# zubair-irshad/articulated-object-nerf

Measured on AMD Instinct MI355X. Metric: rays/sec (64c+128f samples), higher is better.
Workload: dtype f32; 1 GPU; sapien-single-scene vanilla NeRF full-frame render 640x480, 65 coarse + 193 fine evals/ray, 307200 rays per GPU per step, randomized=False, white_bkgd=True; rays_per_gpu=307200, evals_per_ray=258, exchange=none

## Files before the change

### articulated-object-nerf_amd/csrc/aon_mlp.hip

```cpp
#include "aon_pass.h"

namespace aon {

struct VanillaNet {
  static constexpr int kSlotBytes = kPairSlotBytes;
  static constexpr bool kPair = true;
  static constexpr int kNumChunks = aon::kNumChunks;
  static constexpr int chunk_bytes(int c) { return aon::chunk_bytes(c); }
};
struct VanillaFoldNet {
  static constexpr int kSlotBytes = kPairSlotBytes;
  static constexpr bool kPair = true;
  static constexpr int kNumChunks = aon::kNumChunksF;
  static constexpr int chunk_bytes(int c) { return aon::chunk_bytes_f(c); }
};
struct VanillaFoldVbNet {
  static constexpr int kSlotBytes = kPairSlotBytes;
  static constexpr bool kPair = true;
  static constexpr int kNumChunks = aon::kNumChunksF - 1;
  static constexpr int chunk_bytes(int c) { return aon::chunk_bytes_f(c < kChFView ? c : c + 1); }
  static constexpr int skip_before(int c) { return c == kChFView ? kSmallChunkBytes : 0; }
};

struct VanillaTrunkNet {
  static constexpr int kSlotBytes = kPairSlotBytes;
  static constexpr bool kPair = true;
  static constexpr int kNumChunks = kChBott;
  static constexpr int chunk_bytes(int) { return kBigChunkBytes; }
};

struct PackArgs {
  const float* p[kNumVanillaParams];
};

template <bool FOLD>
__global__ void pack_vanilla_kernel(PackArgs a, float* __restrict__ packed, int L, int Lv) {
  const int P = 3 + 6 * L, V = 3 + 6 * Lv;
  const int64_t idx = (int64_t)blockIdx.x * blockDim.x + threadIdx.x;
  constexpr int64_t stream_floats = kStreamBytes / 4;
  constexpr int64_t used_floats = FOLD ? kStreamBytesF / 4 : stream_floats;
  const float* Wf = packed + kFoldTmpOff / 4;
  if (idx >= stream_floats + kSmallFloats) return;
  if (idx >= used_floats && idx < stream_floats) {
    if (idx >= used_floats + 128 * 256 + 128) packed[idx] = 0.f;
    return;
  }
  if (idx >= stream_floats) {
    const int s = (int)(idx - stream_floats);
    float v = 0.f;
    if (s < kSmBiasBott) v = a.p[2 * (s >> 8) + 1][s & 255];
    else if (s < kSmBiasView) v = a.p[19][s - kSmBiasBott];
    else if (s < kSmWSigma) v = FOLD ? Wf[128 * 256 + s - kSmBiasView] : a.p[17][s - kSmBiasView];
    else if (s < kSmWRgb) v = a.p[20][s - kSmWSigma];
    else if (s < kSmBSigma) v = a.p[22][s - kSmWRgb];
    else if (s < kSmBRgb) v = a.p[21][0];
    else if (s < kSmBRgb + 3) v = a.p[23][s - kSmBRgb];
    packed[idx] = v;
    return;
  }
  int c, r, nt;
  constexpr int nbig = FOLD ? kChFView : kNumBigChunks;
  if (idx < (int64_t)nbig * (kBigChunkBytes / 4)) {
    c = (int)(idx / (kBigChunkBytes / 4)); r = (int)(idx % (kBigChunkBytes / 4)); nt = 8;
  } else {
    const int64_t i2 = idx - (int64_t)nbig * (kBigChunkBytes / 4);
    c = nbig + (int)(i2 / (kSmallChunkBytes / 4)); r = (int)(i2 % (kSmallChunkBytes / 4)); nt = 4;
    if constexpr (FOLD) c = c == kChFView ? kChView + 8 : c - 1 + (kChView - kChFView);
  }
  const int cc = r & 3, lane = (r >> 2) & 63, rest = r >> 8;
  const int tp = rest % nt, q = rest / nt;
  const int h = lane >> 5, row = 32 * tp + (lane & 31);
  const float* W; int ld, n_out = 256, col;
  const int hid_col = 8 * q + 4 * h + cc;
  auto pcol = [&](int c63) { return c63 < 0 ? -1 : pos_col_in(c63, L); };
  auto vcol = [&](int c27) { return c27 < 0 ? -1 : view_col_in(c27, Lv); };
  if (c < kChL1) { W = a.p[0]; ld = P; col = pcol(posenc_col(c, q, cc, h)); }
  else if (c < kChL5) { const int l = 1 + (c - kChL1) / 8; W = a.p[2 * l]; ld = 256; col = 32 * ((c - kChL1) % 8) + hid_col; }
  else if (c < kChL5 + 8) { W = a.p[10]; ld = 256 + P; col = 32 * (c - kChL5) + hid_col; }
  else if (c < kChL6) { W = a.p[10]; ld = 256 + P; col = pcol(posenc_col(c - kChL5 - 8, q, cc, h)); if (col >= 0) col += 256; }
  else if (c < kChL7) { W = a.p[12]; ld = 256; col = 32 * (c - kChL6) + hid_col; }
  else if (c < kChBott) { W = a.p[14]; ld = 256; col = 32 * (c - kChL7) + hid_col; }
  else if (c < kChView) { W = a.p[18]; ld = 256; col = 32 * (c - kChBott) + hid_col; }
  else if (c < kChView + 8) {
    W = a.p[16]; ld = 256 + V; n_out = kCondWidth; col = 32 * (c - kChView) + hid_col;
    if constexpr (FOLD) { W = Wf; ld = 256; }
  }
  else { W = a.p[16]; ld = 256 + V; n_out = kCondWidth; col = vcol(viewenc_col(q, cc, h)); if (col >= 0) col += 256; }
  packed[idx] = (col >= 0 && row < n_out) ? W[(int64_t)row * ld + col] : 0.f;
}

struct MlpSeg {
  const char* packed;
  const float* rays_o;
  const float* rays_d;
  const float* viewdirs;
  const float* t_vals;
  const float* samples_enc;
  const float* viewdirs_enc;
  float* raw;
  int64_t total;
  int S;
  int npass;
  union {
    float* planes;
    const int* gather_idx;
    float* live_rows;
  };
  union {
    u32x4* masks;
    const int64_t* gather_count;
    uint8_t* live_mark;
  };
  int64_t Np;
  const float* view_bias;
  static constexpr bool kPerCallBlock = false;
};
struct MlpArgs {
  MlpSeg seg[2];
  int npass_total;
};
__host__ __device__ __forceinline__ const char* seg_stream(const MlpSeg& s) { return s.packed; }
__device__ __forceinline__ const float* seg_small(const MlpSeg& s) { return reinterpret_cast<const float*>(s.packed + kStreamBytes); }

constexpr int kLdsBytes = kRingBytes + (int)kSmallBytes;

struct VanillaTrunk {
  static constexpr int kL0 = kChL0, kL1 = kChL1, kL5 = kChL5, kL6 = kChL6, kL7 = kChL7;
  static constexpr int kBias = kSmBias, kWSigma = kSmWSigma, kBSigma = kSmBSigma, kMask0 = 0;
  static constexpr int plane(int l) { return plane_h(l); }
};

template <bool ENC_IN_KERNEL, bool TRAIN, bool FOLD, bool VB = false, bool GATHER = false, bool DEFER = false>
__global__ void __launch_bounds__(256) mlp_fwd_kernel(MlpArgs args) {
  static_assert(FOLD || !VB, "the per-ray view bias belongs to the folded form");
  static_assert(!GATHER || (ENC_IN_KERNEL && !TRAIN), "the occupancy list serves the inference kernel on in-kernel encodings");
  static_assert(!DEFER || (ENC_IN_KERNEL && !TRAIN && VB && !GATHER), "the deferred view branch serves the dense per-ray-bias inference form");
  using Net = std::conditional_t<DEFER, VanillaTrunkNet, std::conditional_t<VB, VanillaFoldVbNet, std::conditional_t<FOLD, VanillaFoldNet, VanillaNet>>>;
  const int tid = threadIdx.x;
  const int lane = tid & 63, wave = tid >> 6;
  const int m = lane & 31, h = lane >> 5;
  const int wave_s = __builtin_amdgcn_readfirstlane(wave);

  run_passes<Net, kSmallFloats, GATHER>(args, [&](const MlpSeg& sg, int pass, Pipe& p, const float* sm, int64_t listed = 0) __attribute__((always_inline)) {
    int64_t g = (int64_t)pass * 128 + wave * 32 + m;
    bool valid;
    int64_t gc;
    if constexpr (GATHER) {
      valid = g < listed;
      g = gc = sg.gather_idx[valid ? g : listed - 1];
    } else {
      valid = g < sg.total;
      gc = valid ? g : sg.total - 1;
    }
    const int64_t ray = gc / sg.S;

    f32x16 E[2], V;
    float x[3] = {0.f, 0.f, 0.f}, vd[3] = {0.f, 0.f, 0.f};
    if constexpr (ENC_IN_KERNEL) {
      const float t = sg.t_vals[gc];
#pragma unroll
      for (int a = 0; a < 3; ++a) {
        x[a] = __fadd_rn(sg.rays_o[ray * 3 + a], __fmul_rn(t, sg.rays_d[ray * 3 + a]));
        vd[a] = sg.viewdirs[ray * 3 + a];
      }
      encode_pos(x, h, E);
      if constexpr (!VB || TRAIN) encode_view(vd, h, V);
    } else {
      load_pos_enc(sg.samples_enc + gc * kPosEnc, h, E);
      if constexpr (!VB || TRAIN) load_view_enc(sg.viewdirs_enc + ray * kViewEnc, h, V);
    }
    int ray32 = (int)ray;
    (void)ray32;

    PlaneIO io{};
    unsigned moff = 0;
    if constexpr (TRAIN) { io = make_plane_io(sg.planes, kPlRows, (int64_t)pass * 4 + wave_s, m, h); moff = mask_lane_off(pass, tid); }
    if constexpr (TRAIN) {
      store_pos_enc_plane(E, io, kPlE, h);
      store_view_enc_plane(V, io, kPlVE, h);
    }
    FwdTaps<TRAIN, MlpSeg> taps{sg, io, moff};
    f32x16 X[8], Y[8], Z[4];
    auto reread_enc = [&]() {
      if constexpr (TRAIN && !ENC_IN_KERNEL) {
        int64_t gq = gc;
        asm volatile("" : "+v"(gq));
        load_pos_enc(sg.samples_enc + gq * kPosEnc, h, E);
      }
    };
    auto l7_side = [&](auto plain) {
      if constexpr (VB && !DEFER) {
        asm volatile("" : "+v"(ray32));
        return view_bias_side(plain, sg.view_bias + (int64_t)ray32 * kCondWidth + 4 * h, Z);
      } else {
        return plain;
      }
    };
    const float sigma = trunk_fwd<Net, VanillaTrunk>(p, E, X, Y, sm, h, taps, reread_enc, l7_side);
    if constexpr (DEFER) {
      const bool live = sigma > 0.f;
      if (valid) {
        if (h == 0) {
          f32x4 o; o[0] = 0.f; o[1] = 0.f; o[2] = 0.f; o[3] = sigma;
          reinterpret_cast<f32x4*>(sg.raw)[g] = o;
          sg.live_mark[g] = live ? 1 : 0;
        }
        if (live) {
          char* row = reinterpret_cast<char*>(sg.live_rows) + g * 1024 + h * 16;
#pragma unroll
          for (int t = 0; t < 8; ++t) {
#pragma unroll
            for (int q = 0; q < 4; ++q) {
              f32x4 v; v[0] = Y[t][4 * q]; v[1] = Y[t][4 * q + 1]; v[2] = Y[t][4 * q + 2]; v[3] = Y[t][4 * q + 3];
              __builtin_nontemporal_store(v, reinterpret_cast<f32x4*>(row + (32 * t + 8 * q) * 4));
            }
          }
        }
      }
    } else {
      constexpr int kChV = FOLD ? kChFView : kChView;
      auto reencode_view = [&]() {
        if constexpr (TRAIN && ENC_IN_KERNEL) {
          asm volatile("" : "+v"(vd[0]), "+v"(vd[1]), "+v"(vd[2]));
          encode_view(vd, h, V);
        }
        if constexpr (TRAIN && !ENC_IN_KERNEL) {
          int64_t rq = ray;
          asm volatile("" : "+v"(rq));
          load_view_enc(sg.viewdirs_enc + rq * kViewEnc, h, V);
        }
      };
      if constexpr (FOLD) {
        if constexpr (!VB) {
          init_bias(Z, sm + kSmBiasView, h);
          reencode_view();
          chunk_mma<Net, kChV, 4, 14>(p, V, Z);
        }
        dense_layer<Net, kChV + (VB ? 0 : 1), 8, 4>(p, Y, Z, taps.consume(Y, plane_h(7), true)); taps.put_mask(7);
      } else {
        init_bias(X, sm + kSmBiasBott, h); dense_layer<Net, kChBott, 8, 8>(p, Y, X, taps.consume(Y, plane_h(7), true)); taps.put_mask(7);
        init_bias(Z, sm + kSmBiasView, h);
        dense_layer<Net, kChV, 8, 4>(p, X, Z, taps.consume(X, kPlBot, false));
        reencode_view();
        chunk_mma<Net, kChV + 8, 4, 14>(p, V, Z);
      }
      relu_tiles(Z);
      taps.burst(Z, kPlHV, 8);
      float rgb[3];
#pragma unroll
      for (int ch = 0; ch < 3; ++ch) {
        float v = head_partial<4>(Z, sm + kSmWRgb + ch * kCondWidth, h);
        rgb[ch] = v + __shfl_xor(v, 32) + sm[kSmBRgb + ch];
      }
      if (valid && h == 0) {
        f32x4 o; o[0] = rgb[0]; o[1] = rgb[1]; o[2] = rgb[2]; o[3] = sigma;
        reinterpret_cast<f32x4*>(sg.raw)[g] = o;
      }
    }
  });
}

void vanilla_fold_jobs_fwd(const float* const* params, float* packed, int view_levels, FoldGemm jobs[2]) {
  float* Wf = packed + kFoldTmpOff / 4;
  fold_view_jobs(params[16], 256 + 3 + 6 * view_levels, params[17], params[18], params[19], Wf, Wf + 128 * 256, jobs);
}

hipError_t launch_pack_vanilla(const float* const* params, float* packed, hipStream_t stream, int pos_levels, int view_levels, bool fold_done) {
  PackArgs a;
  for (int i = 0; i < kNumVanillaParams; ++i) a.p[i] = params[i];
  const int64_t n = kStreamBytes / 4 + kSmallFloats;
  const int form = fold_default();
  set_stream_form(packed, form);
  if (form == kFormFolded) {
    if (!fold_done) {
      FoldGemm jobs[2];
      vanilla_fold_jobs_fwd(params, packed, view_levels, jobs);
      if (hipError_t e = launch_fold_gemms(jobs, 2, stream); e != hipSuccess) return e;
    }
    pack_vanilla_kernel<true><<<dim3((unsigned)((n + 255) / 256)), dim3(256), 0, stream>>>(a, packed, pos_levels, view_levels);
  } else {
    pack_vanilla_kernel<false><<<dim3((unsigned)((n + 255) / 256)), dim3(256), 0, stream>>>(a, packed, pos_levels, view_levels);
  }
  return hipGetLastError();
}

int num_cus() {
  static std::atomic<int> cache[kMaxDevices];
  int dev = 0;
  if (hipGetDevice(&dev) != hipSuccess) return -1;
  if (dev < 0 || dev >= kMaxDevices) return -1;
  int cus = cache[dev].load(std::memory_order_relaxed);
  if (cus == 0) {
    hipDeviceProp_t prop;
    if (hipGetDeviceProperties(&prop, dev) != hipSuccess) return -1;
    cus = prop.multiProcessorCount;
    cache[dev].store(cus, std::memory_order_relaxed);
  }
  return cus;
}

template <bool ENC, bool TRAIN, bool FOLD, bool VB = false, bool GATHER = false, bool DEFER = false>
static hipError_t launch_mlp_tf(const MlpArgs& args, hipStream_t stream) {
  static DeviceOnce lds_once;
  return launch_persistent(&mlp_fwd_kernel<ENC, TRAIN, FOLD, VB, GATHER, DEFER>, kLdsBytes, args.npass_total, lds_once, stream, args);
}

template <bool ENC, bool TRAIN, bool GATHER = false>
static hipError_t launch_mlp_t(const MlpArgs& args, hipStream_t stream) {
  const int form = agreed_form(args);
  if (form == kFormUnknown) return hipErrorInvalidValue;
  if (args.seg[0].view_bias != nullptr) {
    if constexpr (ENC) return launch_mlp_tf<ENC, TRAIN, true, true, GATHER>(args, stream);
    else return hipErrorInvalidValue;
  }
  return form == kFormFolded ? launch_mlp_tf<ENC, TRAIN, true, false, GATHER>(args, stream)
                             : launch_mlp_tf<ENC, TRAIN, false, false, GATHER>(args, stream);
}

__global__ __launch_bounds__(256) void view_bias_kernel(const float* chunk, const float* bias_vec, const float* viewdirs, int64_t n_rays, float* out) {
  __shared__ float enc[8][2][16];
  const int tid = threadIdx.x;
  const int64_t ray0 = (int64_t)blockIdx.x * 8;
  if (tid < 16) {
    const int64_t ray = ray0 + (tid >> 1);
    if (ray < n_rays) {
      float vd[3] = {viewdirs[ray * 3], viewdirs[ray * 3 + 1], viewdirs[ray * 3 + 2]};
      f32x16 V;
      encode_view(vd, tid & 1, V);
#pragma unroll
      for (int r = 0; r < 16; ++r) enc[tid >> 1][tid & 1][r] = V[r];
    }
  }
  const int row = tid & 127, tp = row >> 5;
  const float bias = bias_vec[row];
  float w[14][2];
#pragma unroll
  for (int r = 0; r < 14; ++r)
#pragma unroll
    for (int hh = 0; hh < 2; ++hh) w[r][hh] = chunk[((((r >> 2) * 4 + tp) * 64 + hh * 32 + (row & 31)) << 2) + (r & 3)];
  __syncthreads();
  for (int k = tid >> 7; k < 8; k += 2) {
    const int64_t ray = ray0 + k;
    if (ray >= n_rays) break;
    float acc = bias;
#pragma unroll
    for (int r = 0; r < 14; ++r) {
      acc = __builtin_fmaf(w[r][0], enc[k][0][r], acc);
      acc = __builtin_fmaf(w[r][1], enc[k][1][r], acc);
    }
    out[ray * kCondWidth + row] = acc;
  }
}

hipError_t launch_view_bias_raw(const float* chunk, const float* bias_vec, const float* viewdirs, int64_t n_rays, float* out, hipStream_t stream) {
  if (n_rays <= 0) return hipSuccess;
  view_bias_kernel<<<dim3((unsigned)((n_rays + 7) / 8)), dim3(256), 0, stream>>>(chunk, bias_vec, viewdirs, n_rays, out);
  return hipGetLastError();
}

hipError_t launch_view_bias(const char* packed, const float* viewdirs, int64_t n_rays, float* out, hipStream_t stream) {
  if (stream_form(packed) != kFormFolded) return hipErrorInvalidValue;
  return launch_view_bias_raw(reinterpret_cast<const float*>(packed + chunk_offset_f(kChFView)), reinterpret_cast<const float*>(packed + kStreamBytes) + kSmBiasView,
                              viewdirs, n_rays, out, stream);
}

struct ViewArgs {
  const char* packed;
  const float* rows;
  const int* idx;
  const int64_t* count;
  const float* view_bias;
  float* raw;
  int S;
};
constexpr int kViewWBytes = 8 * kSmallChunkBytes;
constexpr int kViewLdsBytes = kViewWBytes + (int)kSmallBytes;

__device__ __forceinline__ int view_listed(const ViewArgs& a, int64_t listed, int64_t tile, int m) {
  const int64_t e = tile * 32 + m;
  return a.idx[e < listed ? e : listed - 1];
}
__device__ __forceinline__ void view_gather_tile(const ViewArgs& a, int g, int h, int t, f32x16& Y) {
  const char* row = reinterpret_cast<const char*>(a.rows) + (int64_t)g * 1024 + h * 16;
#pragma unroll
  for (int q = 0; q < 4; ++q) {
    const f32x4 v = *reinterpret_cast<const f32x4*>(row + (32 * t + 8 * q) * 4);
    Y[4 * q] = v[0]; Y[4 * q + 1] = v[1]; Y[4 * q + 2] = v[2]; Y[4 * q + 3] = v[3];
  }
}
__device__ __forceinline__ void view_bias_init(const ViewArgs& a, int g, int h, f32x16 (&Z)[4]) {
  const float* vb = a.view_bias + (int64_t)(g / a.S) * kCondWidth + 4 * h;
#pragma unroll
  for (int i = 0; i < 16; ++i) {
    const f32x4 v = *reinterpret_cast<const f32x4*>(vb + 32 * (i >> 2) + 8 * (i & 3));
    Z[i >> 2][4 * (i & 3)] = v[0]; Z[i >> 2][4 * (i & 3) + 1] = v[1]; Z[i >> 2][4 * (i & 3) + 2] = v[2]; Z[i >> 2][4 * (i & 3) + 3] = v[3];
  }
}
__device__ __forceinline__ void view_chunk(const char* w, int j, int lane, const f32x16& Y, f32x16 (&Z)[4], const f32x16 (&Z0)[4]) {
  const char* buf = w + j * kSmallChunkBytes + lane * 16;
#pragma unroll
  for (int i = 0; i < 16; ++i) {
    const int q = i / 4, tp = i % 4;
    const f32x4 av = *reinterpret_cast<const f32x4*>(buf + i * 1024);
#pragma unroll
    for (int cc = 0; cc < 4; ++cc)
      Z[tp] = __builtin_amdgcn_mfma_f32_32x32x2f32(av[cc], Y[4 * q + cc], (j == 0 && q == 0 && cc == 0) ? Z0[tp] : Z[tp], 0, 0, 0);
  }
}

__global__ void __launch_bounds__(256) view_kernel(ViewArgs a) {
  extern __shared__ __attribute__((aligned(16))) char smem[];
  const int64_t listed = *a.count;
  const int64_t ntiles = (listed + 31) / 32;
  if ((int64_t)blockIdx.x * 4 >= ntiles) return;
  float* sm = reinterpret_cast<float*>(smem + kViewWBytes);
  {
    const f32x4* src = reinterpret_cast<const f32x4*>(a.packed + chunk_offset_f(kChFView + 1));
    f32x4* dst = reinterpret_cast<f32x4*>(smem);
    for (int i = threadIdx.x; i < kViewWBytes / 16; i += 256) dst[i] = src[i];
  }
  load_small_block<kSmallFloats>(sm, reinterpret_cast<const float*>(a.packed + kStreamBytes));
  __syncthreads();
  const int lane = threadIdx.x & 63, m = lane & 31, h = lane >> 5;
  const int wave = __builtin_amdgcn_readfirstlane(threadIdx.x >> 6);
  const int64_t stride = (int64_t)gridDim.x * 4;
  int64_t tile = (int64_t)blockIdx.x * 4 + wave;
  if (tile >= ntiles) return;
  f32x16 Y[8], Z[4], Zb[4];
  int g = view_listed(a, listed, tile, m);
  int gn = view_listed(a, listed, tile + stride, m);
  __builtin_amdgcn_sched_barrier(0);
  view_bias_init(a, g, h, Zb);
  __builtin_amdgcn_sched_barrier(0);
#pragma unroll
  for (int t = 0; t < 8; ++t) view_gather_tile(a, g, h, t, Y[t]);
  __builtin_amdgcn_sched_barrier(0);
  while (true) {
    const int64_t nxt = tile + stride;
    const int gnn = view_listed(a, listed, nxt + stride, m);
#pragma unroll
    for (int j = 0; j < 8; ++j) {
      view_chunk(smem, j, lane, Y[j], Z, Zb);
      __builtin_amdgcn_sched_barrier(0);
      view_gather_tile(a, gn, h, j, Y[j]);
      if (j == 3) view_bias_init(a, gn, h, Zb);
      __builtin_amdgcn_sched_barrier(0);
    }
    relu_tiles(Z);
    float rgb[3];
#pragma unroll
    for (int ch = 0; ch < 3; ++ch) {
      const float v = head_partial<4>(Z, sm + kSmWRgb + ch * kCondWidth, h);
      rgb[ch] = v + __shfl_xor(v, 32) + sm[kSmBRgb + ch];
    }
    if (tile * 32 + m < listed && h == 0) {
      float* rec = a.raw + (int64_t)g * 4;
      rec[0] = rgb[0]; rec[1] = rgb[1]; rec[2] = rgb[2];
    }
    if (nxt >= ntiles) break;
    tile = nxt; g = gn; gn = gnn;
  }
}

hipError_t launch_mlp_trunk_defer(const char* packed, const float* rays_o, const float* rays_d, const float* viewdirs, const float* t_vals,
                                  int64_t n_rays, int S, float* raw, uint8_t* live_mark, float* live_rows, hipStream_t stream) {
  if (stream_form(packed) != kFormFolded) return hipErrorInvalidValue;
  MlpArgs args{};
  fill_seg(args.seg[0], TrainSeg{packed, nullptr, rays_o, rays_d, viewdirs, t_vals, n_rays, S, raw, nullptr, nullptr, 0, nullptr});
  args.seg[0].live_rows = live_rows; args.seg[0].live_mark = live_mark;
  finish_segs(args, 1);
  return launch_mlp_tf<true, false, true, true, false, true>(args, stream);
}

hipError_t launch_view_deferred(const char* packed, const float* live_rows, const int* idx, const int64_t* count, int64_t max_listed,
                                const float* view_bias, int S, float* raw, hipStream_t stream) {
  if (stream_form(packed) != kFormFolded) return hipErrorInvalidValue;
  if (max_listed <= 0) return hipSuccess;
  static DeviceOnce lds_once;
  if (hipError_t e = set_max_lds(&view_kernel, kViewLdsBytes, lds_once); e != hipSuccess) return e;
  const int cus = num_cus();
  if (cus <= 0) return hipErrorInvalidDevice;
  const int64_t groups = (max_listed + 127) / 128;
  const ViewArgs a{packed, live_rows, idx, count, view_bias, raw, S};
  view_kernel<<<dim3((unsigned)(groups < cus ? groups : cus)), dim3(256), kViewLdsBytes, stream>>>(a);
  return hipGetLastError();
}

hipError_t launch_mlp_fwd(const char* packed, const float* rays_o, const float* rays_d, const float* viewdirs,
                          const float* t_vals, int64_t n_rays, int S, float* raw, hipStream_t stream, const float* view_bias) {
  MlpArgs args{};
  fill_seg(args.seg[0], TrainSeg{packed, nullptr, rays_o, rays_d, viewdirs, t_vals, n_rays, S, raw, nullptr, nullptr, 0, view_bias});
  finish_segs(args, 1);
  return launch_mlp_t<true, false>(args, stream);
}

hipError_t launch_mlp_fwd_gather(const char* packed, const float* rays_o, const float* rays_d, const float* viewdirs, const float* t_vals,
                                 int64_t n_rays, int S, float* raw, hipStream_t stream, const float* view_bias, const int* idx, const int64_t* count,
                                 int64_t max_listed) {
  MlpArgs args{};
  MlpSeg& a = args.seg[0];
  fill_seg(a, TrainSeg{packed, nullptr, rays_o, rays_d, viewdirs, t_vals, n_rays, S, raw, nullptr, nullptr, 0, view_bias});
  if (max_listed > 0) a.npass = (int)((max_listed + 127) / 128);
  a.gather_idx = idx; a.gather_count = count;
  finish_segs(args, 1);
  return launch_mlp_t<true, false, true>(args, stream);
}

hipError_t launch_mlp_fwd_train(const char* packed, const float* rays_o, const float* rays_d, const float* viewdirs,
                                const float* t_vals, int64_t n_rays, int S, float* raw, float* planes, void* masks,
                                hipStream_t stream, int64_t np_total, const float* view_bias) {
  const TrainSeg one{packed, nullptr, rays_o, rays_d, viewdirs, t_vals, n_rays, S, raw, planes, masks, np_total, view_bias};
  return launch_mlp_fwd_train2(&one, 1, stream);
}

hipError_t launch_mlp_fwd_train2(const TrainSeg* segs, int nsegs, hipStream_t stream) {
  if (nsegs < 1 || nsegs > 2) return hipErrorInvalidValue;
  MlpArgs args{};
  for (int i = 0; i < nsegs; ++i) fill_seg(args.seg[i], segs[i]);
  finish_segs(args, nsegs);
  return launch_mlp_t<true, true>(args, stream);
}

hipError_t launch_mlp_fwd_train_enc(const char* packed, const float* samples_enc, const float* viewdirs_enc, int64_t n_rays, int S, float* raw,
                                    float* planes, void* masks, hipStream_t stream, int64_t np_total) {
  MlpArgs args{};
  fill_seg(args.seg[0], TrainSeg{packed, nullptr, nullptr, nullptr, nullptr, nullptr, n_rays, S, raw, planes, masks, np_total});
  args.seg[0].samples_enc = samples_enc; args.seg[0].viewdirs_enc = viewdirs_enc;
  finish_segs(args, 1);
  return launch_mlp_t<false, true>(args, stream);
}

hipError_t launch_mlp_fwd_enc(const char* packed, const float* samples_enc, const float* viewdirs_enc,
                              int64_t n_rays, int S, float* raw, hipStream_t stream) {
  MlpArgs args{};
  fill_seg(args.seg[0], TrainSeg{packed, nullptr, nullptr, nullptr, nullptr, nullptr, n_rays, S, raw, nullptr, nullptr, 0});
  args.seg[0].samples_enc = samples_enc; args.seg[0].viewdirs_enc = viewdirs_enc;
  finish_segs(args, 1);
  return launch_mlp_t<false, false>(args, stream);
}


__global__ void __launch_bounds__(256) density_grid_kernel(GridArgs args) {
  const int lane = threadIdx.x & 63, wave = threadIdx.x >> 6;
  const int m = lane & 31, h = lane >> 5;
  run_passes_one<VanillaTrunkNet, kSmallFloats>(args.packed, reinterpret_cast<const float*>(args.packed + kStreamBytes), args.npass,
                                                [&](int pass, Pipe& p, const float* sm) __attribute__((always_inline)) {
    const int64_t l0 = (int64_t)pass * 128 + wave * 32;
    const int64_t l = l0 + m;
    float x[3];
    grid_point(args, l < args.total ? l : args.total - 1, x);
    f32x16 E[2], X[8], Y[8];
    encode_pos(x, h, E);
    NoTaps taps;
    const float sigma = trunk_fwd<VanillaTrunkNet, VanillaTrunk>(p, E, X, Y, sm, h, taps);
    grid_store(args.out, l0, args.total, lane, grid_activation(sigma, args.act));
  });
}

hipError_t launch_density_grid(const char* packed, const int64_t* dims, const float* lo, const float* step, int64_t g_begin, int64_t g_end,
                               int act, float* out, hipStream_t stream) {
  if (stream_form(packed) == kFormUnknown) return hipErrorInvalidValue;
// ... 7 lines not shown
```

### articulated-object-nerf_amd/csrc/aon_mlp_core.h

```cpp
#pragma once
#include "aon_common.h"

#include <type_traits>

namespace aon {

constexpr int kPairSlotBytes = 2 * kBigChunkBytes;
constexpr int kRingBytes = 2 * kPairSlotBytes;

template <class Net> constexpr int pair_offset(int C) { return (C & 1) ? Net::chunk_bytes(C - 1) : 0; }
template <class Net> constexpr int dma_count(int C) {
  return (Net::kNumChunks & 1) ? (C == Net::kNumChunks - 1 ? 2 : (C == Net::kNumChunks - 2 ? 0 : 1)) : 1;
}
template <class Net> constexpr int dma_target(int C, int k) {
  return ((Net::kNumChunks & 1) && C == Net::kNumChunks - 1) ? k : (C + 2) % Net::kNumChunks;
}

template <class Net, class = void> struct NetSkip { static constexpr int at(int) { return 0; } };
template <class Net> struct NetSkip<Net, std::void_t<decltype(Net::skip_before(0))>> { static constexpr int at(int c) { return Net::skip_before(c); } };

struct Pipe {
  const char* stream;
  const char* next_stream;
  char* ring;
// ... 100 lines not shown
    if constexpr (ROUNDS > 0) {
      if (i < ROUNDS) dma_round<Net, C>(p, dma_off, i);
    }
    constexpr int SIDE_PER_STEP = NSTEP >= 16 ? 1 : (16 + NSTEP - 1) / NSTEP;
#pragma unroll
    for (int k = 0; k < SIDE_PER_STEP; ++k) side(i * SIDE_PER_STEP + k);
#pragma unroll
    for (int cc = 0; cc < 4; ++cc) {
      if (4 * q + cc < NREG) {
        if (ZERO_C && q == 0 && cc == 0) {
          const f32x16 zero = {0.f, 0.f, 0.f, 0.f, 0.f, 0.f, 0.f, 0.f, 0.f, 0.f, 0.f, 0.f, 0.f, 0.f, 0.f, 0.f};
          out[tp] = __builtin_amdgcn_mfma_f32_32x32x2f32(a_cur[cc], in[4 * q + cc], zero, 0, 0, 0);
        } else {
          out[tp] = __builtin_amdgcn_mfma_f32_32x32x2f32(a_cur[cc], in[4 * q + cc], out[tp], 0, 0, 0);
        }
      }
    }
    a_cur = a_nxt;
  }
}

template <int NT_OUT>
__device__ __forceinline__ void init_bias(f32x16 (&acc)[NT_OUT], const float* sm_bias, int h) {
#pragma unroll
  for (int tp = 0; tp < NT_OUT; ++tp) {
#pragma unroll
    for (int g = 0; g < 4; ++g) {
      const f32x4 b = *reinterpret_cast<const f32x4*>(sm_bias + 32 * tp + 8 * g + 4 * h);
      acc[tp][4 * g + 0] = b[0]; acc[tp][4 * g + 1] = b[1]; acc[tp][4 * g + 2] = b[2]; acc[tp][4 * g + 3] = b[3];
    }
  }
}

__device__ __forceinline__ float relu1(float x) {
  const int b = __builtin_bit_cast(int, x);
  return __builtin_bit_cast(float, b > 0 ? b : 0);
}

template <int NT>
__device__ __forceinline__ void relu_tiles(f32x16 (&x)[NT]) {
#pragma unroll
  for (int t = 0; t < NT; ++t) {
#pragma unroll
    for (int r = 0; r < 16; ++r) {
      float y = relu1(x[t][r]);
      asm("" : "+v"(y));
      x[t][r] = y;
    }
  }
}

struct NoSideOf {
  __device__ __forceinline__ NoSide operator()(int) const { return NoSide{}; }
};

template <class Net, int CBASE, int NT_IN, int NT_OUT, class SideOf = NoSideOf, bool ZERO_OUT = false>
__device__ __forceinline__ void dense_layer(Pipe& p, const f32x16 (&in)[NT_IN], f32x16 (&out)[NT_OUT], SideOf side_of = SideOf{}) {
  chunk_mma<Net, CBASE + 0, NT_OUT, 16, decltype(side_of(0)), ZERO_OUT>(p, in[0], out, side_of(0));
  chunk_mma<Net, CBASE + 1, NT_OUT, 16>(p, in[1], out, side_of(1));
  chunk_mma<Net, CBASE + 2, NT_OUT, 16>(p, in[2], out, side_of(2));
  chunk_mma<Net, CBASE + 3, NT_OUT, 16>(p, in[3], out, side_of(3));
  if constexpr (NT_IN == 8) {
    chunk_mma<Net, CBASE + 4, NT_OUT, 16>(p, in[4], out, side_of(4));
    chunk_mma<Net, CBASE + 5, NT_OUT, 16>(p, in[5], out, side_of(5));
    chunk_mma<Net, CBASE + 6, NT_OUT, 16>(p, in[6], out, side_of(6));
    chunk_mma<Net, CBASE + 7, NT_OUT, 16>(p, in[7], out, side_of(7));
  }
}

template <int NT>
__device__ __forceinline__ float head_partial(const f32x16 (&x)[NT], const float* sm_w, int h) {
  float acc = 0.f;
#pragma unroll
  for (int t = 0; t < NT; ++t) {
#pragma unroll
    for (int g = 0; g < 4; ++g) {
      const f32x4 w = *reinterpret_cast<const f32x4*>(sm_w + 32 * t + 8 * g + 4 * h);
#pragma unroll
      for (int cc = 0; cc < 4; ++cc) acc = __builtin_fmaf(w[cc], x[t][4 * g + cc], acc);
    }
  }
  return acc;
}


struct PlaneIO {
  char* base;
  unsigned voff;
  unsigned soff;
};

__device__ __forceinline__ PlaneIO make_plane_io(const float* planes, int rows, int64_t step, int m, int h) {
  PlaneIO io;
  int64_t sb = step * (int64_t)rows * 128;
  asm volatile("" : "+s"(sb));
  io.base = const_cast<char*>(reinterpret_cast<const char*>(planes)) + sb;
  io.voff = (unsigned)(h * 512 + m * 16);
  io.soff = (unsigned)(m * 16);
  return io;
}

__device__ __forceinline__ f32x4* quad_ptr(const PlaneIO& io, int row, int g) {
  return reinterpret_cast<f32x4*>(io.base + (int64_t)(row * 128 + g * 1024) + io.voff);
}
__device__ __forceinline__ float* row_ptr(const PlaneIO& io, int row) {
  return reinterpret_cast<float*>(io.base + (int64_t)((row >> 2) * 512 + (row & 3) * 4) + io.soff);
}
template <bool STAGE = true>
__device__ __forceinline__ void store_quad(const PlaneIO& io, int row, int g, const f32x16& t) {
  f32x4 v; v[0] = t[4 * g]; v[1] = t[4 * g + 1]; v[2] = t[4 * g + 2]; v[3] = t[4 * g + 3];
  if constexpr (STAGE)
  asm volatile("" : "+v"(v));
  __builtin_nontemporal_store(v, quad_ptr(io, row, g));
}

typedef unsigned u32x4 __attribute__((ext_vector_type(4)));

__device__ __forceinline__ unsigned mask_lane_off(int pass, int tid) {
  unsigned off = (unsigned)(pass * 256 + tid) * 16u;
  asm volatile("" : "+v"(off));
  return off;
}
template <class T>
__device__ __forceinline__ T* mask_ptr(T* masks, int64_t Np, int slot, unsigned lane_off) {
  int64_t sb = (int64_t)slot * Np * 32;
  asm volatile("" : "+s"(sb));
  using C = std::conditional_t<std::is_const_v<T>, const char, char>;
  return reinterpret_cast<T*>(reinterpret_cast<C*>(masks) + sb + lane_off);
}

__device__ __forceinline__ unsigned mask_push_post(unsigned w, float y_post_relu) {
  const unsigned nb = 0u - __builtin_bit_cast(unsigned, y_post_relu);
  return __builtin_amdgcn_alignbit(w, nb, 31);
}
__device__ __forceinline__ unsigned mask_word_finish(unsigned w) { return __builtin_bitreverse32(w); }

__device__ __forceinline__ float mask_apply(unsigned w, float dh, int pos) {
  int m = __builtin_amdgcn_sbfe((int)w, (unsigned)pos, 1u);
  asm("" : "+v"(m));
  return __builtin_bit_cast(float, __builtin_bit_cast(int, dh) & m);
}

template <int NT>
__device__ __forceinline__ u32x4 relu_mask_bits(const f32x16 (&x)[NT]) {
  u32x4 w = {0u, 0u, 0u, 0u};
#pragma unroll
  for (int t = 0; t < NT; ++t) {
#pragma unroll
    for (int r = 0; r < 16; ++r) w[t >> 1] |= (x[t][r] > 0.f ? 1u : 0u) << ((t & 1) * 16 + r);
  }
  return w;
}

template <int NT>
__device__ __forceinline__ void apply_mask_bits(f32x16 (&x)[NT], const u32x4 w) {
#pragma unroll
  for (int t = 0; t < NT; ++t) {
#pragma unroll
    for (int r = 0; r < 16; ++r) x[t][r] = mask_apply(w[t >> 1], x[t][r], (t & 1) * 16 + r);
  }
}

__device__ __forceinline__ void apply_mask_tile(f32x16& x, const u32x4 w, int t) {
#pragma unroll
  for (int r = 0; r < 16; ++r) x[r] = mask_apply(w[t >> 1], x[r], (t & 1) * 16 + r);
}

template <int NT, bool MASKED, bool STORE = true>
struct BwdSideOf {
  f32x16 (&tiles)[NT];
  int row;
  const PlaneIO& io;
  const u32x4& mk;
  const u32x4* touch = nullptr;
  __device__ __forceinline__ auto operator()(int j) const {
    f32x16 (&t)[NT] = tiles;
    const int trow = row + 32 * j;
    const PlaneIO& pio = io;
    const u32x4& m = mk;
    const u32x4* tch = touch;
    return [&t, trow, &pio, &m, j, tch](int i) {
      if (j == 1 && i == 15 && tch) asm volatile("" ::"v"(*tch));
      if (i < 16) {
        if constexpr (STORE) {
#ifdef AON_CHAIN_STAGE_MASKED
          if ((i & 3) == 0) store_quad<true>(pio, trow, i >> 2, t[j]);
#else
          if ((i & 3) == 0) store_quad<!MASKED>(pio, trow, i >> 2, t[j]);
#endif
        }
        if constexpr (MASKED) {
          if (j + 1 < NT) {
            t[j + 1][i] = mask_apply(m[(j + 1) >> 1], t[j + 1][i], ((j + 1) & 1) * 16 + i);
          }
        }
      }
    };
  }
};

template <int NT>
struct StoreSideOf {
  f32x16 (&tiles)[NT];
  int row;
  const PlaneIO& io;
  __device__ __forceinline__ auto operator()(int j) const {
    f32x16 (&t)[NT] = tiles;
    const int trow = row + 32 * j;
    const PlaneIO& pio = io;
    return [&t, trow, &pio, j](int i) {
      if (i < 16 && (i & 3) == 0) store_quad<false>(pio, trow, i >> 2, t[j]);
    };
  }
};

template <int NT>
__device__ __forceinline__ void store_plane(const f32x16 (&x)[NT], const PlaneIO& io, int row) {
#pragma unroll
  for (int t = 0; t < NT; ++t) {
#pragma unroll
    for (int g = 0; g < 4; ++g) store_quad(io, row + 32 * t, g, x[t]);
  }
}

template <int NT>
__device__ __forceinline__ void load_plane(f32x16 (&x)[NT], const PlaneIO& io, int row) {
#pragma unroll
  for (int t = 0; t < NT; ++t) {
#pragma unroll
    for (int g = 0; g < 4; ++g) {
      const f32x4 v = *quad_ptr(io, row + 32 * t, g);
      x[t][4 * g] = v[0]; x[t][4 * g + 1] = v[1]; x[t][4 * g + 2] = v[2]; x[t][4 * g + 3] = v[3];
    }
  }
}

template <int NT>
__device__ __forceinline__ void zero_tiles(f32x16 (&x)[NT]) {
#pragma unroll
  for (int t = 0; t < NT; ++t)
#pragma unroll
    for (int r = 0; r < 16; ++r) x[t][r] = 0.f;
}

template <bool TRAIN, class Seg>
struct FwdTaps {
  const Seg& sg;
  const PlaneIO& io;
  const unsigned moff;
  unsigned mw[4] = {0u, 0u, 0u, 0u};

  template <int NT>
  __device__ __forceinline__ auto consume(const f32x16 (&in)[NT], int in_row, bool with_mask) {
    return [this, &in, in_row, with_mask](int j) {
      return [this, &in, in_row, with_mask, j](int i) {
        if constexpr (TRAIN) {
          if (i < 16) {
            if ((i & 3) == 0) store_quad<false>(io, in_row + 32 * j, i >> 2, in[j]);
            if (with_mask) mw[j >> 1] = mask_push_post(mw[j >> 1], in[j][i]);
          }
        }
      };
    };
  }
  __device__ __forceinline__ void put_mask(int slot) {
    if constexpr (TRAIN)
      *mask_ptr(sg.masks, sg.Np, slot, moff) = u32x4{mask_word_finish(mw[0]), mask_word_finish(mw[1]), mask_word_finish(mw[2]), mask_word_finish(mw[3])};
    mw[0] = mw[1] = mw[2] = mw[3] = 0u;
  }
  template <int NT>
  __device__ __forceinline__ void burst(const f32x16 (&tiles)[NT], int row, int slot) {
    if constexpr (TRAIN) {
      store_plane(tiles, io, row);
      *mask_ptr(sg.masks, sg.Np, slot, moff) = relu_mask_bits(tiles);
    }
  }
};
struct NoTaps {
  template <int NT> __device__ __forceinline__ NoSideOf consume(const f32x16 (&)[NT], int, bool) const { return NoSideOf{}; }
  __device__ __forceinline__ void put_mask(int) const {}
  template <int NT> __device__ __forceinline__ void burst(const f32x16 (&)[NT], int, int) const {}
};

template <class BaseOf>
__device__ __forceinline__ auto view_bias_side(BaseOf base_of, const float* vb, f32x16 (&Z)[4]) {
  return [base_of, vb, &Z](int j) {
    auto base = base_of(j);
    return [&Z, base, j, vb](int i) {
      base(i);
      if (j == 7 && i < 16) {
        const f32x4 v = *reinterpret_cast<const f32x4*>(vb + 32 * (i >> 2) + 8 * (i & 3));
        Z[i >> 2][4 * (i & 3)] = v[0]; Z[i >> 2][4 * (i & 3) + 1] = v[1]; Z[i >> 2][4 * (i & 3) + 2] = v[2]; Z[i >> 2][4 * (i & 3) + 3] = v[3];
      }
    };
  };
}

struct NoHook {
  __device__ __forceinline__ void operator()() const {}
};
struct PlainSide {
  template <class SideOf> __device__ __forceinline__ SideOf operator()(SideOf s) const { return s; }
};
template <class Net, class T, class Taps, class AtSkip = NoHook, class L7Side = PlainSide>
__device__ __forceinline__ float trunk_fwd(Pipe& p, const f32x16 (&E)[2], f32x16 (&X)[8], f32x16 (&Y)[8], const float* sm, int h, Taps& taps,
                                           AtSkip at_skip = AtSkip{}, L7Side l7_side = L7Side{}) {
  const float* bias = sm + T::kBias;
  init_bias(X, bias + 0 * 256, h);
  chunk_mma<Net, T::kL0 + 0, 8, 16>(p, E[0], X);
  chunk_mma<Net, T::kL0 + 1, 8, 16>(p, E[1], X);
  relu_tiles(X);
  init_bias(Y, bias + 1 * 256, h); dense_layer<Net, T::kL1 + 0, 8, 8>(p, X, Y, taps.consume(X, T::plane(0), true)); taps.put_mask(T::kMask0 + 0); relu_tiles(Y);
  init_bias(X, bias + 2 * 256, h); dense_layer<Net, T::kL1 + 8, 8, 8>(p, Y, X, taps.consume(Y, T::plane(1), true)); taps.put_mask(T::kMask0 + 1); relu_tiles(X);
  init_bias(Y, bias + 3 * 256, h); dense_layer<Net, T::kL1 + 16, 8, 8>(p, X, Y, taps.consume(X, T::plane(2), true)); taps.put_mask(T::kMask0 + 2); relu_tiles(Y);
  init_bias(X, bias + 4 * 256, h); dense_layer<Net, T::kL1 + 24, 8, 8>(p, Y, X, taps.consume(Y, T::plane(3), true)); taps.put_mask(T::kMask0 + 3); relu_tiles(X);
  init_bias(Y, bias + 5 * 256, h);
  dense_layer<Net, T::kL5, 8, 8>(p, X, Y, taps.consume(X, T::plane(4), true)); taps.put_mask(T::kMask0 + 4);
  at_skip();
  chunk_mma<Net, T::kL5 + 8, 8, 16>(p, E[0], Y);
  chunk_mma<Net, T::kL5 + 9, 8, 16>(p, E[1], Y);
  relu_tiles(Y);
  init_bias(X, bias + 6 * 256, h); dense_layer<Net, T::kL6, 8, 8>(p, Y, X, taps.consume(Y, T::plane(5), true)); taps.put_mask(T::kMask0 + 5); relu_tiles(X);
  init_bias(Y, bias + 7 * 256, h);
  dense_layer<Net, T::kL7, 8, 8>(p, X, Y, l7_side(taps.consume(X, T::plane(6), true)));
  taps.put_mask(T::kMask0 + 6); relu_tiles(Y);
  const float sigma = head_partial<8>(Y, sm + T::kWSigma, h);
  return sigma + __shfl_xor(sigma, 32) + sm[T::kBSigma];
}

__device__ __forceinline__ unsigned enc_row_off(int row) { return (unsigned)((row >> 2) * 512 + (row & 3) * 4); }

__device__ __forceinline__ void store_pos_enc_plane(const f32x16 (&E)[2], const PlaneIO& io, int row0, int h) {
  asm volatile("" : "+v"(h));
  char* base = io.base + io.soff;
#pragma unroll
  for (int rho = 0; rho < 30; ++rho) {
    const unsigned off = h ? enc_row_off(row0 + 33 + rho) : enc_row_off(row0 + 3 + rho);
    *reinterpret_cast<float*>(base + off) = E[rho >> 4][rho & 15];
  }
  const unsigned off_id = h ? enc_row_off(row0 + 2) : enc_row_off(row0);
  *reinterpret_cast<float*>(base + off_id) = E[1][14];
  if (!h) *reinterpret_cast<float*>(base + enc_row_off(row0 + 1)) = E[1][15];
}

__device__ __forceinline__ void store_view_enc_plane(const f32x16& V, const PlaneIO& io, int row0, int h) {
  asm volatile("" : "+v"(h));
  char* base = io.base + io.soff;
#pragma unroll
  for (int rho = 0; rho < 12; ++rho) {
    const unsigned off = h ? enc_row_off(row0 + 15 + rho) : enc_row_off(row0 + 3 + rho);
    *reinterpret_cast<float*>(base + off) = V[rho];
  }
  const unsigned off_id = h ? enc_row_off(row0 + 2) : enc_row_off(row0);
  *reinterpret_cast<float*>(base + off_id) = V[12];
  if (!h) *reinterpret_cast<float*>(base + enc_row_off(row0 + 1)) = V[13];
}

__device__ __forceinline__ int pos_col_in(int c63, int L) {
  if (c63 < 3) return c63;
  const bool second = c63 >= 33;
  const int e = second ? c63 - 33 : c63 - 3;
  return e / 3 < L ? 3 + e + (second ? 3 * L : 0) : -1;
}
__device__ __forceinline__ int view_col_in(int c27, int Lv) {
  if (c27 < 3) return c27;
  const bool second = c27 >= 15;
  const int e = second ? c27 - 15 : c27 - 3;
  return e / 3 < Lv ? 3 + e + (second ? 3 * Lv : 0) : -1;
}

__device__ __forceinline__ void encode_pos_scaled(const float (&x)[3], int h, const float* sm_scale, f32x16 (&E)[2]) {
  const float phase = h ? AON_HALF_PI_F32 : 0.f;
  float sc[10];
#pragma unroll
  for (int l = 0; l < 10; ++l) sc[l] = sm_scale[l];
#pragma unroll
  for (int rho = 0; rho < 30; ++rho) {
    const float xb = __fmul_rn(x[rho % 3], sc[rho / 3]);
    E[rho >> 4][rho & 15] = sin_f32(__fadd_rn(xb, phase));
  }
  E[1][14] = h ? x[2] : x[0];
  E[1][15] = h ? 0.f : x[1];
}

__device__ __forceinline__ void encode_pos(const float (&x)[3], int h, f32x16 (&E)[2]) {
  const float phase = h ? AON_HALF_PI_F32 : 0.f;
#pragma unroll
  for (int rho = 0; rho < 30; ++rho) {
    const float xb = __fmul_rn(x[rho % 3], (float)(1 << (rho / 3)));
    E[rho >> 4][rho & 15] = sin_f32(__fadd_rn(xb, phase));
  }
  E[1][14] = h ? x[2] : x[0];
  E[1][15] = h ? 0.f : x[1];
}

__device__ __forceinline__ void encode_view(const float (&vd)[3], int h, f32x16& V) {
  const float phase = h ? AON_HALF_PI_F32 : 0.f;
#pragma unroll
  for (int rho = 0; rho < 12; ++rho) {
    const float xb = __fmul_rn(vd[rho % 3], (float)(1 << (rho / 3)));
    V[rho] = sin_f32(__fadd_rn(xb, phase));
  }
  V[12] = h ? vd[2] : vd[0];
  V[13] = h ? 0.f : vd[1];
  V[14] = 0.f; V[15] = 0.f;
}

__device__ __forceinline__ void load_pos_enc(const float* se, int h, f32x16 (&E)[2]) {
#pragma unroll
  for (int rho = 0; rho < 30; ++rho) E[rho >> 4][rho & 15] = se[3 + rho + 30 * h];
  E[1][14] = h ? se[2] : se[0];
  E[1][15] = h ? 0.f : se[1];
}

__device__ __forceinline__ void load_view_enc(const float* ve, int h, f32x16& V) {
#pragma unroll
  for (int rho = 0; rho < 12; ++rho) V[rho] = ve[3 + rho + 12 * h];
  V[12] = h ? ve[2] : ve[0];
  V[13] = h ? 0.f : ve[1];
  V[14] = 0.f; V[15] = 0.f;
}

__device__ __forceinline__ int posenc_col(int tile, int q, int cc, int h) {
  const int rho = 16 * tile + 4 * q + cc;
  if (rho < 30) return 3 + rho + 30 * h;
  if (rho == 30) return h ? 2 : 0;
  return h ? -1 : 1;
}

__device__ __forceinline__ int viewenc_col(int q, int cc, int h) {
  const int rho = 4 * q + cc;
  if (rho < 12) return 3 + rho + 12 * h;
  if (rho == 12) return h ? 2 : 0;
  if (rho == 13) return h ? -1 : 1;
  return -1;
}


struct GridArgs {
  const char* packed;
  const float* small;
  int64_t ny, nz;
  int64_t g_begin, total;
  float lo[3], step[3];
  int act;
  float* out;
  int npass;
};
inline GridArgs make_grid_args(const char* packed, const float* small, const int64_t* dims, const float* lo, const float* step, int64_t g_begin,
                               int64_t g_end, int act, float* out) {
  GridArgs a{};
  a.packed = packed; a.small = small; a.ny = dims[1]; a.nz = dims[2]; a.g_begin = g_begin; a.total = g_end - g_begin;
  for (int i = 0; i < 3; ++i) { a.lo[i] = lo[i]; a.step[i] = step[i]; }
  a.act = act; a.out = out; a.npass = (int)((a.total + 127) / 128);
  return a;
}

__device__ __forceinline__ void grid_point(const GridArgs& a, int64_t l, float (&x)[3]) {
  const int64_t g = a.g_begin + l;
  const int64_t nyz = a.ny * a.nz;
  const int64_t i = g / nyz, r = g - i * nyz;
  const int64_t j = r / a.nz, k = r - j * a.nz;
  x[0] = __fadd_rn(a.lo[0], __fmul_rn((float)i, a.step[0]));
  x[1] = __fadd_rn(a.lo[1], __fmul_rn((float)j, a.step[1]));
  x[2] = __fadd_rn(a.lo[2], __fmul_rn((float)k, a.step[2]));
}

__device__ __forceinline__ float grid_activation(float raw, int act) {
  if (act == 1) return relu1(raw);
  if (act == 2) return softplus_f32(__fadd_rn(raw, -1.0f));
  return raw;
}

__device__ __forceinline__ void grid_store(float* out, int64_t l0, int64_t total, int lane, float v) {
  const int src = (lane & 7) * 4;
  const float v0 = __shfl(v, src), v1 = __shfl(v, src + 1), v2 = __shfl(v, src + 2), v3 = __shfl(v, src + 3);
  if (lane >= 8) return;
  const int64_t l = l0 + src;
  if (l + 3 < total && (reinterpret_cast<uintptr_t>(out) & 15) == 0) {
    f32x4 o; o[0] = v0; o[1] = v1; o[2] = v2; o[3] = v3;
    *reinterpret_cast<f32x4*>(out + l) = o;
  } else {
    if (l < total) out[l] = v0;
    if (l + 1 < total) out[l + 1] = v1;
    if (l + 2 < total) out[l + 2] = v2;
    if (l + 3 < total) out[l + 3] = v3;
  }
}

}
```

### articulated-object-nerf_amd/csrc/aon_pass.h

```cpp
#pragma once
#include "aon_launch.h"
#include "aon_mlp_core.h"

namespace aon {

template <int SMALL_FLOATS>
__device__ __forceinline__ void load_small_block(float* sm, const float* small) {
  const f32x4* src = reinterpret_cast<const f32x4*>(small);
  f32x4* dst = reinterpret_cast<f32x4*>(sm);
  for (int i = threadIdx.x; i < SMALL_FLOATS / 4; i += 256) dst[i] = src[i];
}

template <class Net, int SMALL_FLOATS, bool GATHER = false, class Args, class Body>
__device__ __forceinline__ void run_passes(const Args& args, Body body) {
  extern __shared__ __attribute__((aligned(16))) char smem[];
  float* sm = reinterpret_cast<float*>(smem + kRingBytes);
  const int lane = threadIdx.x & 63, wave = threadIdx.x >> 6;
  int64_t listed = 0;
  if constexpr (GATHER) listed = *args.seg[0].gather_count;
  const int npass0 = GATHER ? (int)((listed + 127) / 128) : args.seg[0].npass;
  int cur = (int)blockIdx.x >= npass0 ? 1 : 0;
  load_small_block<SMALL_FLOATS>(sm, seg_small(args.seg[cur]));
  Pipe p;
  pipe_init<Net>(p, seg_stream(args.seg[cur]), smem, wave, lane);

  for (int gpass = blockIdx.x; gpass < (GATHER ? npass0 : args.npass_total); gpass += gridDim.x) {
    const int si = gpass >= npass0 ? 1 : 0;
    if (si != cur) {
      __syncthreads();
      load_small_block<SMALL_FLOATS>(sm, seg_small(args.seg[si]));
      __syncthreads();
      cur = si;
    }
    const auto& sg = args.seg[si];
    const int pass = gpass - (si ? npass0 : 0);
    {
      const int nxt = gpass + (int)gridDim.x;
      p.stream = seg_stream(sg);
      p.next_stream = seg_stream(args.seg[(nxt >= npass0 && nxt < (GATHER ? npass0 : args.npass_total)) ? 1 : si]);
    }
    if constexpr (GATHER) body(sg, pass, p, sm, listed);
    else body(sg, pass, p, sm);
  }
  asm volatile("s_waitcnt vmcnt(0)" ::: "memory");
}

template <class Net, int SMALL_FLOATS, class Body>
__device__ __forceinline__ void run_passes_one(const char* stream, const float* small, int npass, Body body) {
  extern __shared__ __attribute__((aligned(16))) char smem[];
  float* sm = reinterpret_cast<float*>(smem + kRingBytes);
  load_small_block<SMALL_FLOATS>(sm, small);
  Pipe p;
  pipe_init<Net>(p, stream, smem, threadIdx.x >> 6, threadIdx.x & 63);
  for (int pass = blockIdx.x; pass < npass; pass += gridDim.x) body(pass, p, sm);
  asm volatile("s_waitcnt vmcnt(0)" ::: "memory");
}

template <class Args>
inline void finish_segs(Args& a, int nsegs) {
  a.npass_total = 0;
  for (int i = 0; i < nsegs; ++i) a.npass_total += a.seg[i].npass;
  if (nsegs == 1) { a.seg[1] = a.seg[0]; a.seg[1].npass = 0; }
  else if (a.seg[0].npass == 0) { a.seg[0] = a.seg[1]; a.seg[1].npass = 0; }
}

template <class Kernel, class Args>
inline hipError_t launch_persistent(Kernel* kernel, int lds_bytes, int npasses, DeviceOnce& once, hipStream_t stream, const Args& args) {
  if (hipError_t e = set_max_lds(kernel, lds_bytes, once); e != hipSuccess) return e;
  const int cus = num_cus();
  if (cus <= 0) return hipErrorInvalidDevice;
  const int grid = npasses < cus ? npasses : cus;
  if (grid <= 0) return hipSuccess;
  kernel<<<dim3(grid), dim3(256), lds_bytes, stream>>>(args);
  return hipGetLastError();
}

template <class Args>
inline int agreed_form(const Args& a) {
  using Seg = std::remove_reference_t<decltype(a.seg[0])>;
  const int form = stream_form(a.seg[0].packed);
  const bool vb = a.seg[0].view_bias != nullptr;
  for (int i = 0; i < 2; ++i) {
    const Seg& s = a.seg[i];
    if (i > 0 && s.npass <= 0) break;
    if (stream_form(s.packed) != form || (s.view_bias != nullptr) != vb) return kFormUnknown;
    if constexpr (Seg::kPerCallBlock) {
      if (stream_form(s.small) != form) return kFormUnknown;
    }
  }
  return vb && form != kFormFolded ? kFormUnknown : form;
}

template <class Seg>
inline void fill_seg(Seg& a, const TrainSeg& t) {
  a.packed = t.packed;
  if constexpr (Seg::kPerCallBlock) a.small = t.small;
  a.rays_o = t.rays_o; a.rays_d = t.rays_d; a.viewdirs = t.viewdirs; a.t_vals = t.t_vals; a.view_bias = t.view_bias;
  a.raw = t.raw; a.total = t.n_rays * t.S; a.S = t.S; a.npass = (int)((a.total + 127) / 128);
  if (t.planes) {
    a.planes = t.planes; a.masks = static_cast<u32x4*>(t.masks); a.Np = t.np_total > 0 ? t.np_total : (int64_t)a.npass * 128;
  }
}

}
```

Baseline: 549,900 rays/s.

## Defer trunk feature-row stores into the next pass's first-layer MMA

In the deferred-view inference kernel, the 1 KB per-sample feature rows and sigma/live-mark heads are no longer written right after the trunk. They are held in a per-thread job and written piecewise during the next pass's first-layer MMA chunk, with a final flush after the loop. Buffer resources with out-of-range offsets replace the branches for masking dead or invalid samples. The aim is to overlap the large global store traffic with matrix compute, at the cost of keeping 128 extra VGPRs of Y alive across passes, which may raise register pressure or cause spills.

```diff
diff --git a/articulated-object-nerf_amd/csrc/aon_mlp.hip b/articulated-object-nerf_amd/csrc/aon_mlp.hip
--- a/articulated-object-nerf_amd/csrc/aon_mlp.hip
+++ b/articulated-object-nerf_amd/csrc/aon_mlp.hip
@@ -130,6 +130,31 @@
   static constexpr int plane(int l) { return plane_h(l); }
 };
 
+struct RowJob {
+  f32x16 Y[8];
+  float sigma;
+  unsigned row_off;
+  int64_t first;
+  int n;
+};
+constexpr unsigned kOutOfBuffer = 0x80000000u;
+constexpr int kBufNt = 2;
+template <class T>
+__device__ __forceinline__ __amdgpu_buffer_rsrc_t job_rsrc(T* base, int64_t first, int n, int bytes_each) {
+  return __builtin_amdgcn_make_buffer_rsrc(reinterpret_cast<char*>(base) + first * bytes_each, 0, n * bytes_each, 0x00020000);
+}
+__device__ __forceinline__ void job_store_heads(const RowJob& job, const MlpSeg& sg, int m, int h) {
+  const bool live = job.sigma > 0.f;
+  f32x4 o; o[0] = 0.f; o[1] = 0.f; o[2] = 0.f; o[3] = job.sigma;
+  __builtin_amdgcn_raw_buffer_store_b128(__builtin_bit_cast(u32x4, o), job_rsrc(sg.raw, job.first, job.n, 16), (int)(h == 0 ? (unsigned)m * 16u : kOutOfBuffer), 0, 0);
+  __builtin_amdgcn_raw_buffer_store_b8((unsigned char)(live ? 1 : 0), job_rsrc(sg.live_mark, job.first, job.n, 1), (int)(h == 0 ? (unsigned)m : kOutOfBuffer), 0, 0);
+}
+__device__ __forceinline__ void job_store_row(const RowJob& job, const MlpSeg& sg, int i) {
+  const int t = i >> 2, q = i & 3;
+  f32x4 v; v[0] = job.Y[t][4 * q]; v[1] = job.Y[t][4 * q + 1]; v[2] = job.Y[t][4 * q + 2]; v[3] = job.Y[t][4 * q + 3];
+  __builtin_amdgcn_raw_buffer_store_b128(__builtin_bit_cast(u32x4, v), job_rsrc(sg.live_rows, job.first, job.n, 1024), (int)(job.row_off + (unsigned)(32 * t + 8 * q) * 4u), 0, kBufNt);
+}
+
 template <bool ENC_IN_KERNEL, bool TRAIN, bool FOLD, bool VB = false, bool GATHER = false, bool DEFER = false>
 __global__ void __launch_bounds__(256) mlp_fwd_kernel(MlpArgs args) {
   static_assert(FOLD || !VB, "the per-ray view bias belongs to the folded form");
@@ -140,6 +165,13 @@
   const int lane = tid & 63, wave = tid >> 6;
   const int m = lane & 31, h = lane >> 5;
   const int wave_s = __builtin_amdgcn_readfirstlane(wave);
+  std::conditional_t<DEFER, RowJob, NoHook> job{};
+  auto flush_slot = [&](int i) __attribute__((always_inline)) {
+    if constexpr (DEFER) {
+      if (i == 0) job_store_heads(job, args.seg[0], m, h);
+      job_store_row(job, args.seg[0], i);
+    }
+  };
 
   run_passes<Net, kSmallFloats, GATHER>(args, [&](const MlpSeg& sg, int pass, Pipe& p, const float* sm, int64_t listed = 0) __attribute__((always_inline)) {
     int64_t g = (int64_t)pass * 128 + wave * 32 + m;
@@ -196,27 +228,26 @@
         return plain;
       }
     };
-    const float sigma = trunk_fwd<Net, VanillaTrunk>(p, E, X, Y, sm, h, taps, reread_enc, l7_side);
-    if constexpr (DEFER) {
-      const bool live = sigma > 0.f;
-      if (valid) {
-        if (h == 0) {
-          f32x4 o; o[0] = 0.f; o[1] = 0.f; o[2] = 0.f; o[3] = sigma;
-          reinterpret_cast<f32x4*>(sg.raw)[g] = o;
-          sg.live_mark[g] = live ? 1 : 0;
-        }
-        if (live) {
-          char* row = reinterpret_cast<char*>(sg.live_rows) + g * 1024 + h * 16;
-#pragma unroll
-          for (int t = 0; t < 8; ++t) {
-#pragma unroll
-            for (int q = 0; q < 4; ++q) {
-              f32x4 v; v[0] = Y[t][4 * q]; v[1] = Y[t][4 * q + 1]; v[2] = Y[t][4 * q + 2]; v[3] = Y[t][4 * q + 3];
-              __builtin_nontemporal_store(v, reinterpret_cast<f32x4*>(row + (32 * t + 8 * q) * 4));
-            }
+    auto l0_side = [&](int j) __attribute__((always_inline)) {
+      return [&flush_slot, j](int i) __attribute__((always_inline)) {
+        if constexpr (DEFER) {
+          if (j == 0) {
+            flush_slot(i);
+            __builtin_amdgcn_sched_barrier(0x786);
           }
         }
-      }
+      };
+    };
+    const float sigma = trunk_fwd<Net, VanillaTrunk>(p, E, X, Y, sm, h, taps, reread_enc, l7_side, l0_side);
+    if constexpr (DEFER) {
+#pragma unroll
+      for (int t = 0; t < 8; ++t) job.Y[t] = Y[t];
+      job.sigma = sigma;
+      job.row_off = sigma > 0.f ? (unsigned)m * 1024u + (unsigned)h * 16u : kOutOfBuffer;
+      asm volatile("" : "+v"(job.row_off));
+      job.first = (int64_t)pass * 128 + wave_s * 32;
+      const int64_t left = sg.total - job.first;
+      job.n = left >= 32 ? 32 : (left > 0 ? (int)left : 0);
     } else {
       constexpr int kChV = FOLD ? kChFView : kChView;
       auto reencode_view = [&]() {
@@ -257,6 +288,9 @@
         reinterpret_cast<f32x4*>(sg.raw)[g] = o;
       }
     }
+  }, [&]() __attribute__((always_inline)) {
+#pragma unroll
+    for (int i = 0; i < 32; ++i) flush_slot(i);
   });
 }
 
diff --git a/articulated-object-nerf_amd/csrc/aon_mlp_core.h b/articulated-object-nerf_amd/csrc/aon_mlp_core.h
--- a/articulated-object-nerf_amd/csrc/aon_mlp_core.h
+++ b/articulated-object-nerf_amd/csrc/aon_mlp_core.h
@@ -426,13 +426,13 @@
 struct PlainSide {
   template <class SideOf> __device__ __forceinline__ SideOf operator()(SideOf s) const { return s; }
 };
-template <class Net, class T, class Taps, class AtSkip = NoHook, class L7Side = PlainSide>
+template <class Net, class T, class Taps, class AtSkip = NoHook, class L7Side = PlainSide, class L0Side = NoSideOf>
 __device__ __forceinline__ float trunk_fwd(Pipe& p, const f32x16 (&E)[2], f32x16 (&X)[8], f32x16 (&Y)[8], const float* sm, int h, Taps& taps,
-                                           AtSkip at_skip = AtSkip{}, L7Side l7_side = L7Side{}) {
+                                           AtSkip at_skip = AtSkip{}, L7Side l7_side = L7Side{}, L0Side l0_side = L0Side{}) {
   const float* bias = sm + T::kBias;
   init_bias(X, bias + 0 * 256, h);
-  chunk_mma<Net, T::kL0 + 0, 8, 16>(p, E[0], X);
-  chunk_mma<Net, T::kL0 + 1, 8, 16>(p, E[1], X);
+  chunk_mma<Net, T::kL0 + 0, 8, 16>(p, E[0], X, l0_side(0));
+  chunk_mma<Net, T::kL0 + 1, 8, 16>(p, E[1], X, l0_side(1));
   relu_tiles(X);
   init_bias(Y, bias + 1 * 256, h); dense_layer<Net, T::kL1 + 0, 8, 8>(p, X, Y, taps.consume(X, T::plane(0), true)); taps.put_mask(T::kMask0 + 0); relu_tiles(Y);
   init_bias(X, bias + 2 * 256, h); dense_layer<Net, T::kL1 + 8, 8, 8>(p, Y, X, taps.consume(Y, T::plane(1), true)); taps.put_mask(T::kMask0 + 1); relu_tiles(X);
diff --git a/articulated-object-nerf_amd/csrc/aon_pass.h b/articulated-object-nerf_amd/csrc/aon_pass.h
--- a/articulated-object-nerf_amd/csrc/aon_pass.h
+++ b/articulated-object-nerf_amd/csrc/aon_pass.h
@@ -11,8 +11,8 @@
   for (int i = threadIdx.x; i < SMALL_FLOATS / 4; i += 256) dst[i] = src[i];
 }
 
-template <class Net, int SMALL_FLOATS, bool GATHER = false, class Args, class Body>
-__device__ __forceinline__ void run_passes(const Args& args, Body body) {
+template <class Net, int SMALL_FLOATS, bool GATHER = false, class Args, class Body, class After = NoHook>
+__device__ __forceinline__ void run_passes(const Args& args, Body body, After after = After{}) {
   extern __shared__ __attribute__((aligned(16))) char smem[];
   float* sm = reinterpret_cast<float*>(smem + kRingBytes);
   const int lane = threadIdx.x & 63, wave = threadIdx.x >> 6;
@@ -42,6 +42,7 @@
     if constexpr (GATHER) body(sg, pass, p, sm, listed);
     else body(sg, pass, p, sm);
   }
+  after();
   asm volatile("s_waitcnt vmcnt(0)" ::: "memory");
 }
 
```

Result: no change. 553,800 rays/s, median of 6 (+0.7%).
